# RocketFlash/EmbeddingNet

Measured on AMD Instinct MI355X. Metric: images/sec training (ResNet18, 224², triplet batch-hard) @ 1/2/4/8 GPU, higher is better.
Workload: dtype f32; 1 GPU; resnet18 224x224x3 synthetic U[0,1), 107-class P x K sampling, local batch 32x4=128 (139 resident batches cycled), E=256, margin 0.5, mining 'hardest' per local batch, radam, fp32 tensors (conv products on 16-bit MFMA from operand splits, fp32 accumulate: 3x3 stride-1 convs and their weight gradients, and the ResNets' other convs where both operands' ranges are known: two fp16 pieces + a per-tenso; global_batch=128, parallelism=dp1, active_triplets_min=192, dead_steps=0, resident_batches=139, step_mode=eager, mining=hardest

## Files before the change

embeddingnet_amd/csrc/conv.hip:

```cpp
#include "gemm_engine.h"
#include "conv_geom.h"
#include "../../include/embnet.h"
#include <stdlib.h>

namespace embnet {

struct InputTransform { const float* scale; const float* shift; int act; };
__device__ __forceinline__ float4 transform4(float4 v, bool ok, const float4& sc, const float4& sh, int act) {
  float4 z = make_float4(fmaf(v.x, sc.x, sh.x), fmaf(v.y, sc.y, sh.y), fmaf(v.z, sc.z, sh.z), fmaf(v.w, sc.w, sh.w));
  if (act == 1) {
    z = make_float4(fmaxf(z.x, 0.f), fmaxf(z.y, 0.f), fmaxf(z.z, 0.f), fmaxf(z.w, 0.f));
  } else if (act == 2) {
    z = make_float4(act_apply(2, z.x), act_apply(2, z.y), act_apply(2, z.z), act_apply(2, z.w));
  }
  return ok ? z : make_float4(0.f, 0.f, 0.f, 0.f);
}


template <int ROWS, bool VEC, bool TF = false>
struct LoadConvFwdA {
  using Tile = TileKC<ROWS>;
  static constexpr bool CAN_INTERLEAVE = VEC && !TF;
  Buf buf; int H, W, C, Kg; FastDiv dC, dS; int tid;
  unsigned base[Tile::PASSES]; int ih0[Tile::PASSES], iw0[Tile::PASSES];
// ... 268 lines not shown
#pragma unroll
      for (int r = 0; r < 16; ++r) acc[i][j][r] = (acc[i][j][r] * fb) * fa;
}

struct SplitTail { int n_full, parts, kt_part; float* ws; };

struct ConvFwdParams { const float* x; const float* w; const float* bias; float* y; ConvGeom g; int relu; SplitTail tail; const float* residual; InputTransform tf; float* stats; int stats_rows; int fair_from; Ranges rg; };

template <class G>
__device__ __forceinline__ void tail_decode(const SplitTail& t, int bid, int kt_total, int& tile, int& k0, int& k1,
                                            float*& part) {
  if (bid < t.n_full) { tile = xcd_remap(bid, t.n_full); k0 = 0; k1 = kt_total; part = nullptr; return; }
  const int j = bid - t.n_full;
  tile = t.n_full + j / t.parts;
  k0 = (j % t.parts) * t.kt_part; k1 = min(kt_total, k0 + t.kt_part);
  part = t.ws + (long)j * (G::BM * G::BN);
}

template <class G>
__device__ __forceinline__ void store_partial(const f32x16 (&acc)[G::TM][G::TN], float* smem, float* part) {
  for_each_acc_row4<G>(acc, smem, [&](int r, int c, float4 v) {
    *reinterpret_cast<float4*>(part + r * G::BN + c) = v;
  });
}


__device__ __forceinline__ void bn_sums_add(int act, float4 v, float4 xq, float4 sc, float4 sh, float4 mu, float4 rs,
                                            float4& s1, float4& s2, float4& s3) {
  float4 dz = v;
  if (act) {
    dz.x = act_grad(act, fmaf(xq.x, sc.x, sh.x), v.x); dz.y = act_grad(act, fmaf(xq.y, sc.y, sh.y), v.y);
    dz.z = act_grad(act, fmaf(xq.z, sc.z, sh.z), v.z); dz.w = act_grad(act, fmaf(xq.w, sc.w, sh.w), v.w);
  }
  s3.x = fmaxf(s3.x, fabsf(dz.x)); s3.y = fmaxf(s3.y, fabsf(dz.y)); s3.z = fmaxf(s3.z, fabsf(dz.z)); s3.w = fmaxf(s3.w, fabsf(dz.w));
  s1.x += dz.x; s1.y += dz.y; s1.z += dz.z; s1.w += dz.w;
  s2.x = fmaf(dz.x, (xq.x - mu.x) * rs.x, s2.x); s2.y = fmaf(dz.y, (xq.y - mu.y) * rs.y, s2.y);
  s2.z = fmaf(dz.z, (xq.z - mu.z) * rs.z, s2.z); s2.w = fmaf(dz.w, (xq.w - mu.w) * rs.w, s2.w);
}

__global__ __launch_bounds__(256) void tail_fixup_kernel(const float* __restrict__ ws, int parts, int bm, int bn, int wtm,
                                                         int n_full, int tiles_n, long m, int cols,
                                                         const float* __restrict__ bias, int relu,
                                                         const float* __restrict__ residual, float* __restrict__ out,
                                                         float* __restrict__ stats, int stats_rows, const BnSums bsum) {
  __shared__ float4 red[3][256];
  const int cpb = 1024 / wtm, qpb = cpb / 4;
  const int blocks_per_tile = bm * bn / 1024, col_groups = bn / cpb;
  const int t = blockIdx.x / blocks_per_tile, bi = blockIdx.x % blocks_per_tile;
  const int band = bi / col_groups, cg = bi % col_groups;
  const int rr = threadIdx.x / qpb, r = band * wtm + rr, c = cg * cpb + (threadIdx.x % qpb) * 4;
  const int tile = n_full + t;
  const long row = (long)(tile / tiles_n) * bm + r;
  const int col = (tile % tiles_n) * bn + c;
  const bool in = row < m && col < cols;
  float4 a = make_float4(0.f, 0.f, 0.f, 0.f);
  if (in) {
    const float* src = ws + (long)t * parts * bm * bn + r * bn + c;
    a = *reinterpret_cast<const float4*>(src);
    for (int k = 1; k < parts; ++k) {
      const float4 v = *reinterpret_cast<const float4*>(src + (long)k * bm * bn);
// ... 963 lines not shown
```

embeddingnet_amd/csrc/conv_geom.h:

```cpp
#pragma once
#include "common.h"

namespace embnet {

struct FastDiv {
  uint32_t mul, shift, d;
  static FastDiv make(uint32_t d) {
    FastDiv f; f.d = d;
    uint32_t s = 0; while ((1ull << s) < d) ++s;
    f.shift = s;
    f.mul = (uint32_t)((((1ull << s) - d) << 32) / d + 1);
    return f;
  }
  __device__ __forceinline__ uint32_t div(uint32_t n) const { return (__umulhi(n, mul) + n) >> shift; }
  __device__ __forceinline__ void divmod(uint32_t n, uint32_t& q, uint32_t& r) const { q = div(n); r = n - q * d; }
};

struct ConvGeom {
  int N, H, W, C, R, S, K, stride, pad_t, pad_l, OH, OW;
  FastDiv dOHW, dOW, dHW, dW, dC, dK, dS;
};

constexpr int ROW_INVALID = -(1 << 28);
constexpr size_t CONV_MAX_OPERAND_BYTES = 0x7FFFFFF0ull;


__device__ __forceinline__ void split_k(int kk, const FastDiv& dinner, const FastDiv& dS, int& r, int& s, int& c) {
  uint32_t rs, cc; dinner.divmod((uint32_t)kk, rs, cc);
  uint32_t rr, ss; dS.divmod(rs, rr, ss);
  r = (int)rr; s = (int)ss; c = (int)cc;
}

struct BnSums { const float* x; const float* scale; const float* shift; const float* mean; const float* rstd; int act; float* partial; int rows; int kinds; };
constexpr BnSums NO_BN_SUMS = BnSums{nullptr, nullptr, nullptr, nullptr, nullptr, 0, nullptr, 0};

void launch_tail_fixup(const float* ws, int parts, int bm, int bn, int wtm, int n_full, int rem, int tiles_n, long m, int cols,
                       const float* bias, int relu, const float* residual, float* out, float* stats, int stats_rows,
                       const BnSums& bsum, hipStream_t st);
void launch_slab_reduce(const float* slabs, int splits, long n, float* out, hipStream_t st);

bool thin_gemm_applies(int red, int ncols);
int thin_gemm_stats_rows(long m, int ncols);
int launch_thin_gemm(const float* in, const float* w, int w_transposed, long m, int red, int ncols, float* out, float* stats,
                     const float* bias, int relu, const float* residual, int stride, int n, int h, int wd, int oh, int ow, hipStream_t st);

bool thin_wgrad_applies(int c, int k);
int thin_wgrad_splits(long m, int c, int k);
int launch_thin_wgrad(const float* x, const float* dy, float* slabs, long m, int c, int k, int stride, int n, int h, int wd, int oh,
                      int ow, hipStream_t st);

inline int make_geom(ConvGeom& g, int n, int h, int w, int c, int r, int s, int k, int stride, int pad_t,
                     int pad_l, int oh, int ow, const char* who) {
  EMBNET_CHECK_ARG(n > 0 && h > 0 && w > 0 && c > 0 && r > 0 && s > 0 && k > 0 && stride > 0 && oh > 0 && ow > 0,
                   "%s: non-positive dimension", who);
  EMBNET_CHECK_ARG(pad_t >= 0 && pad_l >= 0, "%s: negative padding", who);
  EMBNET_CHECK_ARG((oh - 1) * stride + 1 - pad_t <= h && (ow - 1) * stride + 1 - pad_l <= w,
                   "%s: output %dx%d reaches outside the %dx%d input", who, oh, ow, h, w);
  EMBNET_CHECK_ARG((size_t)n * h * w * c * 4 <= CONV_MAX_OPERAND_BYTES && (size_t)n * oh * ow * k * 4 <= CONV_MAX_OPERAND_BYTES &&
// ... 12 lines not shown
```

embeddingnet_amd/csrc/conv_patch.hip:

```cpp
#include "gemm_engine.h"
#include "conv_geom.h"
#include "../../include/embnet.h"

namespace embnet {
namespace patch {

typedef __attribute__((address_space(3))) void* lds_ptr;
__device__ __forceinline__ void dma16(__amdgpu_buffer_rsrc_t r, unsigned char* lds, unsigned voff, unsigned soff) {
  __builtin_amdgcn_raw_ptr_buffer_load_lds(r, (lds_ptr)lds, 16, (int)voff, (int)soff, 0, 0);
}

template <int BN_>
struct GeomP {
  static constexpr int BM = 256, BN = BN_, WAVES_M = 4, WAVES_N = 2, WTM = 64, WTN = BN_ / 2, TM = 2, TN = WTN / 32;
};

struct PatchParams {
  const unsigned short* xp;
  const unsigned short* wp;
  float* y; const float* bias; const float* residual; float* stats; int stats_rows; int relu;
  ConvGeom g; unsigned x_plane_bytes, w_plane_bytes;
  int PH, PW; FastDiv dPHW, dPW;
  int LR;
  int n_full, parts, cc_part, n_pieces, grid; float* ws;
// ... 31 lines not shown
  kargp pp = kargs();
  FastDiv dOHW, dOW;
  dOHW.mul = pp->g.dOHW.mul; dOHW.shift = pp->g.dOHW.shift; dOHW.d = pp->g.dOHW.d;
  dOW.mul = pp->g.dOW.mul; dOW.shift = pp->g.dOW.shift; dOW.d = pp->g.dOW.d;
  uint32_t n, rem, oh, ow;
  dOHW.divmod((uint32_t)m, n, rem); dOW.divmod(rem, oh, ow);
  return (int)n * (pp->PH * pp->PW) + (int)oh * pp->PW + (int)ow;
}

template <class G, bool F16, int NP>
__device__ __forceinline__ void step_planes(const bf16x8 (&a)[G::TM][NP], const bf16x8 (&b)[G::TN][NP], f32x16 (&acc)[G::TM][G::TN]) {
  if constexpr (F16) {
    f16x8 ah[G::TM][2], bh[G::TN][2];
#pragma unroll
    for (int i = 0; i < G::TM; ++i) { ah[i][0] = __builtin_bit_cast(f16x8, a[i][0]); ah[i][1] = __builtin_bit_cast(f16x8, a[i][1]); }
#pragma unroll
    for (int i = 0; i < G::TN; ++i) { bh[i][0] = __builtin_bit_cast(f16x8, b[i][0]); bh[i][1] = __builtin_bit_cast(f16x8, b[i][1]); }
    mfma_step_h<G::TM, G::TN>(ah, bh, acc);
  } else {
    mfma_step3<G>(a, b, acc);
  }
}

template <class G, int BN, bool BNS, bool F16>
__device__ __forceinline__ void patch_epilogue(const PatchParams& p, const Item& cur, f32x16 (&acc)[G::TM][G::TN], int M, int K,
                                               int wave, int lane, int h, int wm, int wn) {
  constexpr int TM = G::TM, TN = G::TN;
  if (F16) {
    const float osx = p.a_range ? scale_pair(scale_exponent_of(__uint_as_float(*p.a_range))).y
                                : planes_scale_slot(p.xp, (long)(p.x_plane_bytes >> 1))[1];
    const float osw = planes_scale_slot(p.wp, (long)(p.w_plane_bytes >> 1))[1];
#pragma unroll
    for (int im = 0; im < TM; ++im)
#pragma unroll
      for (int in = 0; in < TN; ++in)
#pragma unroll
        for (int rr = 0; rr < 16; ++rr) acc[im][in][rr] = (acc[im][in][rr] * osw) * osx;
  }
  if (cur.part) {
    float* part = cur.part + (wm + 4 * h) * BN + wn + (lane & 31);
#pragma unroll
    for (int im = 0; im < TM; ++im)
#pragma unroll
      for (int in = 0; in < TN; ++in)
#pragma unroll
        for (int rr = 0; rr < 16; ++rr)
          part[(im * 32 + (rr & 3) + 8 * (rr >> 2)) * BN + in * 32] = acc[im][in][rr];
  } else {
    const bool inner = cur.m0 + 256 <= M && cur.n0 + BN <= K;
#pragma unroll
    for (int in = 0; in < TN; ++in) {
      const int col = cur.n0 + wn + in * 32 + (lane & 31);
      const bool cok = col < K;
      const float bv = (p.bias && cok) ? p.bias[col] : 0.f;
      float s1 = 0.f, s2 = 0.f;
      constexpr bool bnm = BNS;
      float bsc = 0.f, bsh = 0.f, bmu = 0.f, brs = 0.f;
      float ev[BNS ? TM : 1][16];
      if (BNS) {
        if (cok) { bsc = p.bn.scale[col]; bsh = p.bn.shift[col]; bmu = p.bn.mean[col]; brs = p.bn.rstd[col]; }
#pragma unroll
        for (int im = 0; im < TM; ++im) {
          const long o0 = (long)(cur.m0 + wm + im * 32 + 4 * h) * K + col;
#pragma unroll
          for (int rr = 0; rr < 16; ++rr) {
            const int row = cur.m0 + wm + im * 32 + (rr & 3) + 8 * (rr >> 2) + 4 * h;
            ev[BNS ? im : 0][rr] = (inner || (row < M && cok)) ? p.bn.x[o0 + (long)((rr & 3) + 8 * (rr >> 2)) * K] : 0.f;
          }
        }
      }
#pragma unroll
      for (int im = 0; im < TM; ++im) {
        const long o0 = (long)(cur.m0 + wm + im * 32 + 4 * h) * K + col;
        float v[16];
#pragma unroll
        for (int rr = 0; rr < 16; ++rr) { v[rr] = acc[im][in][rr] + bv; if (p.relu) v[rr] = fmaxf(v[rr], 0.f); }
        if (inner) {
          if (p.residual) {
#pragma unroll
            for (int rr = 0; rr < 16; ++rr) v[rr] += p.residual[o0 + (long)((rr & 3) + 8 * (rr >> 2)) * K];
          }
#pragma unroll
          for (int rr = 0; rr < 16; ++rr) {
            p.y[o0 + (long)((rr & 3) + 8 * (rr >> 2)) * K] = v[rr];
            if (BNS) {
              const float e = ev[BNS ? im : 0][rr], dz = act_grad(p.bn.act, fmaf(e, bsc, bsh), v[rr]);
              s1 += dz; s2 = fmaf(dz, (e - bmu) * brs, s2);
            } else { s1 += v[rr]; s2 = fmaf(v[rr], v[rr], s2); }
          }
        } else {
#pragma unroll
          for (int rr = 0; rr < 16; ++rr) {
            const int row = cur.m0 + wm + im * 32 + (rr & 3) + 8 * (rr >> 2) + 4 * h;
            if (row < M && cok) {
              const long o = o0 + (long)((rr & 3) + 8 * (rr >> 2)) * K;
              if (p.residual) v[rr] += p.residual[o];
              p.y[o] = v[rr];
              if (BNS) {
                const float e = ev[BNS ? im : 0][rr], dz = act_grad(p.bn.act, fmaf(e, bsc, bsh), v[rr]);
                s1 += dz; s2 = fmaf(dz, (e - bmu) * brs, s2);
              } else { s1 += v[rr]; s2 = fmaf(v[rr], v[rr], s2); }
            }
          }
        }
      }
      if (p.stats || bnm) {
        s1 += __shfl_xor(s1, 32, 64); s2 += __shfl_xor(s2, 32, 64);
        if (h == 0 && cok) {
          float* const dst = bnm ? p.bn.partial : p.stats;
          const long prow = (long)cur.tile_m * G::WAVES_M + wave / G::WAVES_N, P = bnm ? p.bn.rows : p.stats_rows;
          dst[(long)col * P + prow] = s1;
          dst[((long)K + col) * P + prow] = s2;
        }
      }
    }
  }

}

template <int BN, int R, int S, int TPS, int NBS, bool BNS = false, bool F16 = false, bool PIPE = false>
__global__ __launch_bounds__(640) void conv_patch_kernel(const PatchParams p) {
  using G = GeomP<BN>;
  constexpr int NP = F16 ? 2 : 3;
  constexpr int TM = G::TM, TN = G::TN, SPC = R * S / TPS, D = NBS - 1;
  constexpr int SBY = TPS * NP * BN * 32;
  constexpr int NBI = TPS * NP * (BN / 32);
  static_assert((R * S) % TPS == 0 && SPC >= 2, "steps per chunk");
  extern __shared__ __attribute__((aligned(16))) unsigned char smem[];
  const int tid = threadIdx.x, lane = tid & 63, h = lane >> 5;
  const int wave = __builtin_amdgcn_readfirstlane(tid >> 6);
  const int LR = p.LR, PLP = LR * 32, PB = NP * PLP;
  unsigned char* const bslot0 = smem + 2 * PB;
  const int b = blockIdx.x;
  const int n_mine = b < p.n_full ? (p.n_full - b + p.grid - 1) / p.grid : 0;
  const int n_items = n_mine + (b < p.n_pieces ? 1 : 0);
  if (n_items == 0) return;
  const int dhalf = (lane & 1) ^ ((lane >> 4) & 1);

  if (wave == 8) {
    const __amdgpu_buffer_rsrc_t wr = __builtin_amdgcn_make_buffer_rsrc(const_cast<unsigned short*>(p.wp), 0, 3u * p.w_plane_bytes, 0x00020000);
    const int K = p.g.K, NCC = p.g.C / 16;
    const unsigned wpb = p.w_plane_bytes;
    int it = 0; Item t = work_item<BN>(0, n_mine);
    int cc = t.cc_b, st = 0; bool live = true;
// ... 16 lines not shown
        for (int q = 0; q < NP; ++q)
#pragma unroll
          for (int gb = 0; gb < BN / 32; ++gb)
            dma16(wr, slot + ((tp * NP + q) * BN + gb * 32) * 32, live ? rowoff[gb] : OOB, q * wpb + so);
      }
      if (live && ++st == SPC) {
        st = 0;
        if (++cc == t.cc_e) {
          if (++it < n_items) { t = work_item<BN>(it, n_mine); cc = t.cc_b; tile_rows(); } else live = false;
        }
      }
    };
    int total = 0;
    for (int i = 0; i < n_items; ++i) { const Item q = work_item<BN>(i, n_mine); total += (q.cc_e - q.cc_b) * SPC; }
    for (int gs = 0; gs < D; ++gs) issue(gs);
    for (int gs = 0; gs < total; ++gs) {
      asm volatile("s_waitcnt vmcnt(%0)" :: "n"((D - 1) * NBI) : "memory");
      __builtin_amdgcn_s_barrier();
      issue(gs + D);
    }
    asm volatile("s_waitcnt vmcnt(0)" ::: "memory");
    return;
  }
  if (wave == 9) {
    const __amdgpu_buffer_rsrc_t xr = __builtin_amdgcn_make_buffer_rsrc(const_cast<unsigned short*>(p.xp), 0, 3u * p.x_plane_bytes, 0x00020000);
    const int NG = LR / 32;
    const unsigned xpb = p.x_plane_bytes, chunk_bytes = 32u * (unsigned)(p.g.N * p.g.H * p.g.W);
    unsigned poff[16];
    auto tile_offsets = [&](const Item& t) {
      kargp pp = kargs();
      FastDiv dPHW, dPW;
      dPHW.mul = pp->dPHW.mul; dPHW.shift = pp->dPHW.shift; dPHW.d = pp->dPHW.d;
      dPW.mul = pp->dPW.mul; dPW.shift = pp->dPW.shift; dPW.d = pp->dPW.d;
      const int P0 = padded_pos(t.m0), N = pp->g.N, H = pp->g.H, W = pp->g.W, pt = pp->g.pad_t, pl = pp->g.pad_l;
#pragma unroll
      for (int gI = 0; gI < 16; ++gI) {
        const int idx = P0 + 32 * gI + (lane >> 1);
        uint32_t n, rem, py, px;
        dPHW.divmod((uint32_t)idx, n, rem); dPW.divmod(rem, py, px);
        const int ih = (int)py - pt, iw = (int)px - pl;
        const bool ok = gI < NG && (int)n < N && (unsigned)ih < (unsigned)H && (unsigned)iw < (unsigned)W;
        poff[gI] = ok ? 32u * (unsigned)(((int)n * H + ih) * W + iw) + 16u * dhalf : OOB;
      }
    };
    auto issue = [&](int cc, int gc) {
      unsigned char* buf = smem + (gc & 1) * PB;
// ... 106 lines not shown
          const int tap = st * TPS + tp, r = tap / S, s = tap % S;
          bf16x8 a[TM][NP], bb[TN][NP];
#pragma unroll
          for (int im = 0; im < TM; ++im) {
            const int idx = rowidx[im] + r * PW + s;
            const unsigned char* ap = pbuf + idx * 32 + ((h ^ ((idx >> 3) & 1)) << 4);
#pragma unroll
            for (int q = 0; q < NP; ++q) a[im][q] = *reinterpret_cast<const bf16x8*>(ap + q * PLP);
          }
#pragma unroll
          for (int in = 0; in < TN; ++in) {
            const int row = wn + in * 32 + (lane & 31);
            const unsigned char* bp = bs + (tp * NP * BN + row) * 32 + ((h ^ ((row >> 3) & 1)) << 4);
#pragma unroll
            for (int q = 0; q < NP; ++q) bb[in][q] = *reinterpret_cast<const bf16x8*>(bp + q * BN * 32);
          }
          step_planes<G, F16>(a, bb, acc);
          if (TPS > 1) __builtin_amdgcn_sched_barrier(0);
        }
        ++gs;
      }
      ++gc;
    }
    patch_epilogue<G, BN, BNS, F16>(p, cur, acc, M, K, wave, lane, h, wm, wn);
  }
}

template <int BN, int G, int NS, bool F16>
__global__ __launch_bounds__(704) void conv1x1_planes_kernel(const PatchParams p) {
  using GP = GeomP<BN>;
  static_assert(F16, "the 1x1 planes kernel is built for the two-piece fp16 format");
  constexpr int NP = 2, TM = GP::TM, TN = GP::TN, D = NS - 1;
  constexpr int A_BYTES = G * NP * 256 * 32, B_BYTES = G * NP * BN * 32, STAGE = A_BYTES + B_BYTES;
  constexpr int NBI_B = G * NP * (BN / 32), NBI_A = NP * 8;
  extern __shared__ __attribute__((aligned(16))) unsigned char smem[];
  const int tid = threadIdx.x, lane = tid & 63, h = lane >> 5;
  const int wave = __builtin_amdgcn_readfirstlane(tid >> 6);
  const int b = blockIdx.x;
  const int n_mine = b < p.n_full ? (p.n_full - b + p.grid - 1) / p.grid : 0;
  const int n_items = n_mine + (b < p.n_pieces ? 1 : 0);
  if (n_items == 0) return;
  const int dhalf = (lane & 1) ^ ((lane >> 4) & 1);
  int total = 0;
  for (int i = 0; i < n_items; ++i) { const Item q = work_item<BN, 16 * G>(i, n_mine); total += q.cc_e - q.cc_b; }

  if (wave >= 8) {
    const bool is_b = wave == 8;
    const int tp = wave - 9;
// ... 89 lines not shown
        for (int q = 0; q < 2; ++q) {
#pragma unroll
          for (int im = 0; im < TM; ++im) a[im][q] = *reinterpret_cast<const f16x8*>(sa + (c2 * NP + q) * 256 * 32 + aoff[im]);
#pragma unroll
          for (int in = 0; in < TN; ++in) bb[in][q] = *reinterpret_cast<const f16x8*>(sb + (c2 * NP + q) * BN * 32 + boff[in]);
        }
      };
      load(0, fa[0], fb[0]);
      __builtin_amdgcn_sched_barrier(0);
#pragma unroll
      for (int c2 = 0; c2 < G; ++c2) {
        if (c2 + 1 < G) load(c2 + 1, fa[(c2 + 1) & 1], fb[(c2 + 1) & 1]);
        mfma_step_h<TM, TN>(fa[c2 & 1], fb[c2 & 1], acc);
        constexpr int NMF = 3 * TM * TN, NRD = 2 * (TM + TN);
#pragma unroll
        for (int i = 0; i < NMF; ++i) {
          __builtin_amdgcn_sched_group_barrier(0x008, 1, 0);
          if (c2 + 1 < G && i < NRD) __builtin_amdgcn_sched_group_barrier(0x100, 1, 0);
        }
        __builtin_amdgcn_sched_barrier(0);
      }
      ++gs;
    }
    patch_epilogue<GP, BN, false, F16>(p, cur, acc, M, K, wave, lane, h, wm, wn);
  }
}

template <int BN>
__global__ __launch_bounds__(704) void conv1x1_a32_kernel(const PatchParams p) {
  using GP = GeomP<BN>;
  constexpr int G = 2, NS = 3, NP = 2, TM = GP::TM, TN = GP::TN, D = NS - 1;
  constexpr int A_BYTES = 256 * 128, B_BYTES = G * NP * BN * 32, STAGE = A_BYTES + B_BYTES;
  constexpr int NBI_B = G * NP * (BN / 32), NBI_A = 16;
  extern __shared__ __attribute__((aligned(16))) unsigned char smem[];
  const int tid = threadIdx.x, lane = tid & 63, h = lane >> 5;
  const int wave = __builtin_amdgcn_readfirstlane(tid >> 6);
  const int b = blockIdx.x;
  const int n_mine = b < p.n_full ? (p.n_full - b + p.grid - 1) / p.grid : 0;
  const int n_items = n_mine + (b < p.n_pieces ? 1 : 0);
  if (n_items == 0) return;
  int total = 0;
  for (int i = 0; i < n_items; ++i) { const Item q = work_item<BN, 16 * G>(i, n_mine); total += q.cc_e - q.cc_b; }

  if (wave >= 8) {
    const bool is_b = wave == 8;
    const int tp = wave - 9;
    const __amdgpu_buffer_rsrc_t rs = is_b
// ... 98 lines not shown
        for (int q = 0; q < 2; ++q)
#pragma unroll
          for (int in = 0; in < TN; ++in) bb[in][q] = *reinterpret_cast<const f16x8*>(sb + (c2 * NP + q) * BN * 32 + boff[in]);
      };
      auto split = [&](f16x8 (&a)[TM][2]) {
        typedef uint32_t u32x4 __attribute__((ext_vector_type(4)));
#pragma unroll
        for (int im = 0; im < TM; ++im) {
          const Split4H s0 = split4h(raw[im][0], a_scale), s1 = split4h(raw[im][1], a_scale);
          a[im][0] = __builtin_bit_cast(f16x8, u32x4{s0.p[0].x, s0.p[0].y, s1.p[0].x, s1.p[0].y});
          a[im][1] = __builtin_bit_cast(f16x8, u32x4{s0.p[1].x, s0.p[1].y, s1.p[1].x, s1.p[1].y});
        }
      };
      load_raw(0); load_b(0, fb[0]);
      split(fa[0]);
#pragma unroll
      for (int c2 = 0; c2 < G; ++c2) {
        if (c2 + 1 < G) { load_raw(c2 + 1); load_b(c2 + 1, fb[(c2 + 1) & 1]); }
        mfma_step_h<TM, TN>(fa[c2 & 1], fb[c2 & 1], acc);
        if (c2 + 1 < G) split(fa[(c2 + 1) & 1]);
      }
      ++gs;
    }
    patch_epilogue<GP, BN, false, true>(p, cur, acc, M, K, wave, lane, h, wm, wn);
  }
}

struct WPlanesTensor { const float* w; unsigned short* out; int R, S, C, K, flip, pad; };
static_assert(sizeof(WPlanesTensor) == 40, "descriptor layout is part of the ABI (include/embnet.h)");
__global__ __launch_bounds__(256) void weight_planes_kernel(const WPlanesTensor* __restrict__ table, const int* __restrict__ chunks, int f16) {
  const WPlanesTensor t = table[chunks[2 * blockIdx.x]];
  const int rows = t.flip ? t.C : t.K, red = t.flip ? t.K : t.C, ncc = red / 16;
  const long plane = (long)t.R * t.S * t.C * t.K, total4 = plane / 4;
  const long i = (long)chunks[2 * blockIdx.x + 1] * 1024 + threadIdx.x;
#pragma unroll
  for (int u = 0; u < 4; ++u) {
    const long i4 = i + u * 256;
    if (i4 >= total4) return;
    long e = 4 * i4;
    const int j = (int)(e % 16); e /= 16;
    const int row = (int)(e % rows); e /= rows;
    const int s = (int)(e % t.S); e /= t.S;
    const int cc = (int)(e % ncc); const int r = (int)(e / ncc);
    float v[4];
#pragma unroll
    for (int q = 0; q < 4; ++q) {
      const int ch = cc * 16 + j + q;
// ... 227 lines not shown
                              void* workspace, size_t workspace_bytes, void* stream, const char* who) {
  const ConvGeom& g = p.g;
  const long M = (long)g.N * g.OH * g.OW;
  p.stats_rows = cdiv(M, 256) * 4;
  p.grid = pl.grid;
  if (pl.n_pieces > 0 && (pl.ws_bytes > workspace_bytes || !workspace)) { pl.n_full = pl.tiles; pl.n_pieces = 0; pl.parts = 1; }
  p.n_full = pl.n_full; p.parts = pl.parts; p.cc_part = pl.cc_part; p.n_pieces = pl.n_pieces; p.ws = (float*)workspace;
  hipStream_t st = (hipStream_t)stream;
  {
    EMBNET_TRACE_FLOP(kname, 2.0 * M * g.K * g.R * g.S * g.C, operand_bytes + 4.0 * (double)M * g.K * (p.residual ? 2 : 1), st);
    launch(p, pl, st);
  }
  if (p.n_pieces > 0)
    launch_tail_fixup(p.ws, p.parts, 256, pl.bn, 64, p.n_full, pl.tiles - p.n_full, cdiv(g.K, pl.bn), M, g.K, p.bias, p.relu, p.residual,
                      p.y, p.stats, p.stats_rows, p.bn, st);
  return check_launch(who);
}

template <int BN, int TPS, int NBS>
static void launch_patch_as(const PatchParams& p, size_t lds, hipStream_t st) {
  if (!p.bn.x) {
    if (planes_f16()) launch_planes<conv_patch_kernel<BN, 3, 3, TPS, NBS, false, true, true>>(p, 640, lds, st);
    else launch_planes<conv_patch_kernel<BN, 3, 3, TPS, NBS, false, false>>(p, 640, lds, st);
  } else if (!planes_f16()) launch_planes<conv_patch_kernel<BN, 3, 3, TPS, NBS, true, false>>(p, 640, lds, st);
  else launch_planes<conv_patch_kernel<BN, 3, 3, TPS, NBS, true, true>>(p, 640, lds, st);
}
static void launch_patch(const PatchParams& p, const Plan& pl, hipStream_t st) {
  if (pl.bn == 128 && pl.tps == 3) { if (pl.nbs == 3) launch_patch_as<128, 3, 3>(p, pl.lds, st); else launch_patch_as<128, 3, 2>(p, pl.lds, st); }
  else if (pl.bn == 128) { if (pl.nbs == 6) launch_patch_as<128, 1, 6>(p, pl.lds, st); else launch_patch_as<128, 1, 4>(p, pl.lds, st); }
  else launch_patch_as<64, 3, 3>(p, pl.lds, st);
}

static int conv2d_patch_impl(const void* xp, const void* wp, const float* bias, float* y, int n, int h, int wd, int c,
                             int r, int s, int k, int pad_t, int pad_l, int oh, int ow, int relu,
                             const float* residual, float* stats, const BnSums& bsum, void* workspace, size_t workspace_bytes,
                             void* stream) {
  EMBNET_CHECK_ARG(xp && wp && y, "conv2d_patch: null pointer");
  EMBNET_CHECK_ARG(r == 3 && s == 3, "conv2d_patch: 3x3 kernels (1x1: embnet_conv2d_planes1x1_f32)");
  Plan pl;
  EMBNET_CHECK_ARG(make_plan(n, c, r, s, k, 1, oh, ow, pl), "conv2d_patch: unsupported geometry (see embnet_conv2d_patch_supported)");
  PatchParams p{(const unsigned short*)xp, (const unsigned short*)wp, y, bias, residual, stats, 0, relu};
  if (int rc = make_geom(p.g, n, h, wd, c, r, s, k, 1, pad_t, pad_l, oh, ow, "conv2d_patch")) return rc;
  p.x_plane_bytes = (unsigned)((size_t)n * h * wd * c * 2);
  p.w_plane_bytes = (unsigned)((size_t)r * s * c * k * 2);
  p.PH = oh + r - 1; p.PW = ow + s - 1;
  p.dPHW = FastDiv::make(p.PH * p.PW); p.dPW = FastDiv::make(p.PW);
  p.LR = pl.LR;
  p.bn = bsum;
  static thread_local char kname[160];
  snprintf(kname, sizeof kname, "void embnet::patch::conv_patch_kernel<%d, 3, 3, %d, %d, %s%s>(embnet::patch::PatchParams)", pl.bn, pl.tps, pl.nbs,
           p.bn.x ? "true" : "false", planes_f16() ? (p.bn.x ? ", true" : ", true, true") : "");
  return launch_planes_gemm(p, pl, kname, (planes_f16() ? 4.0 : 6.0) * ((double)n * h * wd * c + (double)r * s * c * k), launch_patch,
                            workspace, workspace_bytes, stream, "conv2d_patch");
}

extern "C" int embnet_conv2d_patch_f32(const void* xp, const void* wp, const float* bias, float* y, int n, int h, int wd, int c,
                                       int r, int s, int k, int pad_t, int pad_l, int oh, int ow, int relu,
                                       const float* residual, float* stats, void* workspace, size_t workspace_bytes,
                                       void* stream) {
  return conv2d_patch_impl(xp, wp, bias, y, n, h, wd, c, r, s, k, pad_t, pad_l, oh, ow, relu, residual, stats, NO_BN_SUMS, workspace,
                           workspace_bytes, stream);
}

static void fill_1x1(PatchParams& p) {
  const ConvGeom& g = p.g;
  p.w_plane_bytes = (unsigned)((size_t)g.C * g.K * 2);
  p.PH = g.OH; p.PW = g.OW; p.dPHW = FastDiv::make(g.OH * g.OW); p.dPW = FastDiv::make(g.OW);
  p.LR = 256;
  p.bn = NO_BN_SUMS;
}

static void launch_1x1(const PatchParams& p, const Plan& pl, hipStream_t st) {
  if (pl.bn == 128) launch_planes<conv1x1_planes_kernel<128, ONE_G, ONE_NS, true>>(p, 704, pl.lds, st);
  else launch_planes<conv1x1_planes_kernel<64, ONE_G, ONE_NS, true>>(p, 704, pl.lds, st);
// ... 22 lines not shown
  else launch_planes<conv1x1_a32_kernel<64>>(p, 704, pl.lds, st);
}
extern "C" int embnet_conv2d_dma1x1_supported(int n, int h, int wd, int c, int k, int stride, int oh, int ow) {
  Plan pl;
  return dma1x1_ok(n, h, wd, c, k, stride, oh, ow, pl) ? 1 : 0;
}
extern "C" int embnet_conv2d_dma1x1_f32(const float* x, const void* wp, const float* bias, float* y, int n, int h, int wd, int c, int k,
                                        int stride, int oh, int ow, int relu, const float* residual, float* stats,
                                        const uint32_t* x_range, void* workspace, size_t workspace_bytes, void* stream) {
  EMBNET_CHECK_ARG(x && wp && y && x_range, "conv2d_dma1x1: null pointer (the activation's range slot is required)");
  EMBNET_CHECK_ARG(!(reinterpret_cast<uintptr_t>(x) & 15) && !(reinterpret_cast<uintptr_t>(x_range) & 3), "conv2d_dma1x1: alignment");
  Plan pl;
  EMBNET_CHECK_ARG(dma1x1_ok(n, h, wd, c, k, stride, oh, ow, pl), "conv2d_dma1x1: unsupported geometry (embnet_conv2d_dma1x1_supported)");
  PatchParams p{(const unsigned short*)x, (const unsigned short*)wp, y, bias, residual, stats, 0, relu};
  if (int rc = make_geom(p.g, n, h, wd, c, 1, 1, k, stride, 0, 0, oh, ow, "conv2d_dma1x1")) return rc;
  p.x_plane_bytes = 0; p.x32_bytes = (unsigned)((size_t)n * h * wd * c * 4); p.a_range = x_range;
  fill_1x1(p);
  static thread_local char kname[160];
  snprintf(kname, sizeof kname, "void embnet::patch::conv1x1_a32_kernel<%d>(embnet::patch::PatchParams)", pl.bn);
  return launch_planes_gemm(p, pl, kname, 4.0 * ((double)n * oh * ow * c + (double)c * k), launch_dma1x1, workspace, workspace_bytes, stream,
                            "conv2d_dma1x1");
}

extern "C" int embnet_conv2d_patch_bnsums_f32(const void* xp, const void* wp, float* y, int n, int h, int wd, int c, int r, int s, int k,
                                              int pad_t, int pad_l, int oh, int ow, const float* bn_x, const float* bn_scale,
                                              const float* bn_shift, const float* bn_mean, const float* bn_rstd, int bn_act,
                                              float* bn_partial, int bn_rows, void* workspace, size_t workspace_bytes, void* stream) {
  EMBNET_CHECK_ARG(bn_x && bn_scale && bn_shift && bn_mean && bn_rstd && bn_partial, "conv2d_patch_bnsums: null pointer");
  EMBNET_CHECK_ARG(bn_act >= 0 && bn_act <= 2, "conv2d_patch_bnsums: activation code %d", bn_act);
  EMBNET_CHECK_ARG(bn_rows > 0 && bn_rows == embnet_conv2d_patch_stats_rows(n, oh, ow),
                   "conv2d_patch_bnsums: rows %d for this geometry (see embnet_conv2d_patch_stats_rows)", bn_rows);
  return conv2d_patch_impl(xp, wp, nullptr, y, n, h, wd, c, r, s, k, pad_t, pad_l, oh, ow, 0, nullptr, nullptr,
                           BnSums{bn_x, bn_scale, bn_shift, bn_mean, bn_rstd, bn_act, bn_partial, bn_rows}, workspace, workspace_bytes, stream);
}
```

embeddingnet_amd/layers.py:

```python
import contextlib
import math
import os as _os

import torch
from torch import nn

from . import _lib
from ._lib import check, ptr, stream


def env_switch(var, default):
    return {"0": False, "1": True}.get(_os.environ.get(var), default)


@contextlib.contextmanager
def switches(**values):
    old = {name: globals()[name][0] for name in values}
    try:
        for name, v in values.items():
            globals()[name][0] = v
        yield
    finally:
        for name, v in old.items():
            globals()[name][0] = v
# ... 448 lines not shown
    return base.as_strided(tuple(shape), (0,) * len(shape), 1)


def _is_placeholder(t):
    return (t.dim() == 4 and t.numel() > 1 and t.stride() == (0, 0, 0, 0) and t.storage_offset() == 1
            and t.untyped_storage().nbytes() == 12)


def _take_dy_planes(dy):
    e = DY_PLANES.pop(dy.data_ptr(), None)
    return e[0] if (e is not None and e[1].shape == dy.shape) else None


def patch_ok(n, h, wd, c, r, s, k, stride, oh, ow):
    return bool(_lib.lib().embnet_conv2d_patch_supported(n, c, r, s, k, stride, oh, ow))


def _patch_dgrad(dy_planes, w, dx, n, h, wd, c, r, s, k, pt, pl, oh, ow, dx_add, bn_src=None):
    lib = _lib.lib()
    ws = workspace(lib.embnet_conv2d_patch_workspace_bytes(n, k, r, s, c, h, wd), dx.device)
    if bn_src is not None and dx_add is None and PATCH_BN_SUMS[0]:
        bn_x, bn_stats, bn_act = bn_src
        rows = lib.embnet_conv2d_patch_stats_rows(n, h, wd)
        partial = torch.empty((2, c, rows), device=dx.device, dtype=torch.float32)
        st = _StatsRows(bn_stats)
        check(lib.embnet_conv2d_patch_bnsums_f32(ptr(dy_planes), ptr(weight_planes(w, 1)), ptr(dx), n, oh, ow, k, r, s, c,
                                                 r - 1 - pt, s - 1 - pl, h, wd, ptr(bn_x), st.scale, st.shift, st.mean, st.rstd,
                                                 int(bn_act), ptr(partial), rows, ptr(ws), ws.numel() * 4, stream()))
        BN_SUMS.put(dx.data_ptr(), (partial, rows, bn_x.data_ptr(), dx.detach()), 8, "oldest")
        return
    check(lib.embnet_conv2d_patch_f32(ptr(dy_planes), ptr(weight_planes(w, 1)), None, ptr(dx), n, oh, ow, k, r, s, c,
                                      r - 1 - pt, s - 1 - pl, h, wd, 0, ptr(dx_add), None, ptr(ws), ws.numel() * 4, stream()))


STATS_ROWS = ("mean", "rstd", "scale", "shift", "bound", "range", "xhat")
STATS_HEIGHTS = (4, 6, 7)


class _StatsRows:
    __slots__ = STATS_ROWS

    def __init__(self, stats):
        p, height, row = stats.data_ptr(), stats.shape[0], 4 * stats.shape[1]
        self.mean, self.rstd, self.scale, self.shift = p, p + row, p + 2 * row, p + 3 * row
        self.bound, self.range = (p + 4 * row, p + 5 * row) if height >= 6 else (None, None)
        self.xhat = p + 6 * row if height >= 7 else None


def _in_affine(in_stats):
    st = _StatsRows(in_stats) if in_stats is not None else None
    return (st.scale, st.shift) if st is not None else (None, None)
# ... 1689 lines not shown
```

include/embnet.h:

```cpp
#ifndef EMBNET_H
#define EMBNET_H

#include <stddef.h>
#include <stdint.h>

#ifdef __cplusplus
extern "C" {
#endif

#define EMBNET_ABI_VERSION 22

enum {
  EMBNET_MINE_SEMIHARD = 0,
  EMBNET_MINE_HARDEST = 1,
  EMBNET_MINE_RANDOM_HARD = 2,
  EMBNET_MINE_BATCH_HARD = 3
};

int embnet_abi_version(void);
const char* embnet_last_error(void);

int embnet_trace_enable(int on);
int embnet_trace_reset(void);
int embnet_trace_count(void);
// ... 143 lines not shown
int embnet_conv1x1_thin_supported(int red, int ncols);

int embnet_conv2d_patch_supported(int n, int c, int r, int s, int k, int stride, int oh, int ow);
size_t embnet_conv2d_patch_workspace_bytes(int n, int c, int r, int s, int k, int oh, int ow);
int embnet_conv2d_patch_stats_rows(int n, int oh, int ow);
int embnet_conv2d_patch_f32(const void* x_planes, const void* w_planes, const float* bias, float* y, int n, int h, int wd, int c,
                            int r, int s, int k, int pad_t, int pad_l, int oh, int ow, int relu, const float* residual,
                            float* stats, void* workspace, size_t workspace_bytes, void* stream);
int embnet_conv2d_stem_supported(int n, int h, int wd, int c, int r, int s, int k, int stride, int pad_t, int pad_l, int oh, int ow);
int embnet_conv2d_stem_stats_rows(int n, int oh, int ow);
int embnet_conv2d_stem_f32(const float* x, const float* w, float* y, int n, int h, int wd, int pad_t, int pad_l, int oh, int ow,
                           float* stats, const uint32_t* x_range, const uint32_t* w_range, void* stream);
int embnet_conv2d_planes1x1_f32(const void* x_planes, const void* w_planes, const float* bias, float* y, int n, int h, int wd, int c,
                                int k, int stride, int oh, int ow, int relu, const float* residual, float* stats,
                                void* workspace, size_t workspace_bytes, void* stream);
int embnet_conv2d_dma1x1_supported(int n, int h, int wd, int c, int k, int stride, int oh, int ow);
int embnet_conv2d_dma1x1_f32(const float* x, const void* wp, const float* bias, float* y, int n, int h, int wd, int c, int k,
                             int stride, int oh, int ow, int relu, const float* residual, float* stats, const uint32_t* x_range,
                             void* workspace, size_t workspace_bytes, void* stream);
int embnet_conv2d_patch_bnsums_f32(const void* x_planes, const void* w_planes, float* y, int n, int h, int wd, int c, int r, int s,
                                   int k, int pad_t, int pad_l, int oh, int ow, const float* bn_x, const float* bn_scale,
                                   const float* bn_shift, const float* bn_mean, const float* bn_rstd, int bn_act,
                                   float* bn_partial, int bn_rows, void* workspace, size_t workspace_bytes, void* stream);
int embnet_se_mlp_supported(int n, int c, int s);
int embnet_se_mlp_fwd(const float* pooled, const float* w1, const float* b1, const float* w2, const float* b2, int n, int c, int s,
                      float* z1, float* gate, void* stream);
int embnet_se_mlp_bwd(const float* dgate, const float* gate, const float* z1, const float* pooled, const float* w1, const float* w2,
                      int n, int c, int s, float* dz1, float* dpooled, float* dw1, float* db1, float* dw2, float* db2, void* stream);
int embnet_planes_from_f32(const float* x, long pixels, int c, void* planes, void* stream);
int embnet_conv_weight_planes_chunk_elems(void);
int embnet_conv_weight_planes(const void* table, int n_tensors, const int32_t* chunks, int n_chunks, void* stream);
int embnet_affine_act_planes(const float* x, long m, int c, const float* scale, const float* shift, int act, float* y,
                             void* planes, void* stream);
int embnet_affine_act_planes_ex(const float* x, long m, int c, const float* scale, const float* shift, int act, float* y,
                                void* planes, const float* y_bound, uint32_t* y_range, void* stream);
int embnet_conv2d_wgrad_planes_supported(int n, int h, int wd, int c, int r, int s, int k, int stride, int pad_t, int pad_l,
                                         int oh, int ow);
int embnet_conv2d_wgrad_planes_splits(int n, int h, int wd, int c, int k);
size_t embnet_conv2d_wgrad_planes_workspace_bytes(int n, int h, int wd, int c, int k);
int embnet_conv2d_wgrad_planes_f32(const void* x_planes, const void* dy_planes, float* dw, void* workspace,
                                   size_t workspace_bytes, int n, int h, int wd, int c, int k, int reduce, void* stream);

int embnet_u8_to_f32(const void* src, const int32_t* index, int n, long pixels, int c_in, int c_out, float denom, float* dst,
                     void* stream);

size_t embnet_augment_param_floats(void);
// ... 257 lines not shown
```

Before: 16820 images/sec.

## Move BN-backward sums out of patch conv epilogue into dedicated sums waves

The fused dgrad+BN-sums patch kernel no longer computes batch-norm backward reductions inside the MFMA waves' epilogue. Two extra waves (768 threads) stream back the freshly written dx tile plus the BN input and accumulate sum, weighted sum and a new max|dz| statistic, running one tile behind the compute waves. The aim is to take the extra reads and ALU work off the GEMM critical path and overlap them with the next tile's math. The cost is more barriers and higher register and occupancy pressure. It also adds a third partial-stats plane that the Python caller now allocates and requests.

```diff
diff --git a/embeddingnet_amd/csrc/conv.hip b/embeddingnet_amd/csrc/conv.hip
--- a/embeddingnet_amd/csrc/conv.hip
+++ b/embeddingnet_amd/csrc/conv.hip
@@ -314,20 +314,6 @@
   for_each_acc_row4<G>(acc, smem, [&](int r, int c, float4 v) {
     *reinterpret_cast<float4*>(part + r * G::BN + c) = v;
   });
-}
-
-
-__device__ __forceinline__ void bn_sums_add(int act, float4 v, float4 xq, float4 sc, float4 sh, float4 mu, float4 rs,
-                                            float4& s1, float4& s2, float4& s3) {
-  float4 dz = v;
-  if (act) {
-    dz.x = act_grad(act, fmaf(xq.x, sc.x, sh.x), v.x); dz.y = act_grad(act, fmaf(xq.y, sc.y, sh.y), v.y);
-    dz.z = act_grad(act, fmaf(xq.z, sc.z, sh.z), v.z); dz.w = act_grad(act, fmaf(xq.w, sc.w, sh.w), v.w);
-  }
-  s3.x = fmaxf(s3.x, fabsf(dz.x)); s3.y = fmaxf(s3.y, fabsf(dz.y)); s3.z = fmaxf(s3.z, fabsf(dz.z)); s3.w = fmaxf(s3.w, fabsf(dz.w));
-  s1.x += dz.x; s1.y += dz.y; s1.z += dz.z; s1.w += dz.w;
-  s2.x = fmaf(dz.x, (xq.x - mu.x) * rs.x, s2.x); s2.y = fmaf(dz.y, (xq.y - mu.y) * rs.y, s2.y);
-  s2.z = fmaf(dz.z, (xq.z - mu.z) * rs.z, s2.z); s2.w = fmaf(dz.w, (xq.w - mu.w) * rs.w, s2.w);
 }
 
 __global__ __launch_bounds__(256) void tail_fixup_kernel(const float* __restrict__ ws, int parts, int bm, int bn, int wtm,
diff --git a/embeddingnet_amd/csrc/conv_geom.h b/embeddingnet_amd/csrc/conv_geom.h
--- a/embeddingnet_amd/csrc/conv_geom.h
+++ b/embeddingnet_amd/csrc/conv_geom.h
@@ -34,6 +34,19 @@
 struct BnSums { const float* x; const float* scale; const float* shift; const float* mean; const float* rstd; int act; float* partial; int rows; int kinds; };
 constexpr BnSums NO_BN_SUMS = BnSums{nullptr, nullptr, nullptr, nullptr, nullptr, 0, nullptr, 0};
 
+__device__ __forceinline__ void bn_sums_add(int act, float4 v, float4 xq, float4 sc, float4 sh, float4 mu, float4 rs,
+                                            float4& s1, float4& s2, float4& s3) {
+  float4 dz = v;
+  if (act) {
+    dz.x = act_grad(act, fmaf(xq.x, sc.x, sh.x), v.x); dz.y = act_grad(act, fmaf(xq.y, sc.y, sh.y), v.y);
+    dz.z = act_grad(act, fmaf(xq.z, sc.z, sh.z), v.z); dz.w = act_grad(act, fmaf(xq.w, sc.w, sh.w), v.w);
+  }
+  s3.x = fmaxf(s3.x, fabsf(dz.x)); s3.y = fmaxf(s3.y, fabsf(dz.y)); s3.z = fmaxf(s3.z, fabsf(dz.z)); s3.w = fmaxf(s3.w, fabsf(dz.w));
+  s1.x += dz.x; s1.y += dz.y; s1.z += dz.z; s1.w += dz.w;
+  s2.x = fmaf(dz.x, (xq.x - mu.x) * rs.x, s2.x); s2.y = fmaf(dz.y, (xq.y - mu.y) * rs.y, s2.y);
+  s2.z = fmaf(dz.z, (xq.z - mu.z) * rs.z, s2.z); s2.w = fmaf(dz.w, (xq.w - mu.w) * rs.w, s2.w);
+}
+
 void launch_tail_fixup(const float* ws, int parts, int bm, int bn, int wtm, int n_full, int rem, int tiles_n, long m, int cols,
                        const float* bias, int relu, const float* residual, float* out, float* stats, int stats_rows,
                        const BnSums& bsum, hipStream_t st);
diff --git a/embeddingnet_amd/csrc/conv_patch.hip b/embeddingnet_amd/csrc/conv_patch.hip
--- a/embeddingnet_amd/csrc/conv_patch.hip
+++ b/embeddingnet_amd/csrc/conv_patch.hip
@@ -77,7 +77,7 @@
   }
 }
 
-template <class G, int BN, bool BNS, bool F16>
+template <class G, int BN, bool F16>
 __device__ __forceinline__ void patch_epilogue(const PatchParams& p, const Item& cur, f32x16 (&acc)[G::TM][G::TN], int M, int K,
                                                int wave, int lane, int h, int wm, int wn) {
   constexpr int TM = G::TM, TN = G::TN;
@@ -109,21 +109,6 @@
       const bool cok = col < K;
       const float bv = (p.bias && cok) ? p.bias[col] : 0.f;
       float s1 = 0.f, s2 = 0.f;
-      constexpr bool bnm = BNS;
-      float bsc = 0.f, bsh = 0.f, bmu = 0.f, brs = 0.f;
-      float ev[BNS ? TM : 1][16];
-      if (BNS) {
-        if (cok) { bsc = p.bn.scale[col]; bsh = p.bn.shift[col]; bmu = p.bn.mean[col]; brs = p.bn.rstd[col]; }
-#pragma unroll
-        for (int im = 0; im < TM; ++im) {
-          const long o0 = (long)(cur.m0 + wm + im * 32 + 4 * h) * K + col;
-#pragma unroll
-          for (int rr = 0; rr < 16; ++rr) {
-            const int row = cur.m0 + wm + im * 32 + (rr & 3) + 8 * (rr >> 2) + 4 * h;
-            ev[BNS ? im : 0][rr] = (inner || (row < M && cok)) ? p.bn.x[o0 + (long)((rr & 3) + 8 * (rr >> 2)) * K] : 0.f;
-          }
-        }
-      }
 #pragma unroll
       for (int im = 0; im < TM; ++im) {
         const long o0 = (long)(cur.m0 + wm + im * 32 + 4 * h) * K + col;
@@ -138,10 +123,7 @@
 #pragma unroll
           for (int rr = 0; rr < 16; ++rr) {
             p.y[o0 + (long)((rr & 3) + 8 * (rr >> 2)) * K] = v[rr];
-            if (BNS) {
-              const float e = ev[BNS ? im : 0][rr], dz = act_grad(p.bn.act, fmaf(e, bsc, bsh), v[rr]);
-              s1 += dz; s2 = fmaf(dz, (e - bmu) * brs, s2);
-            } else { s1 += v[rr]; s2 = fmaf(v[rr], v[rr], s2); }
+            s1 += v[rr]; s2 = fmaf(v[rr], v[rr], s2);
           }
         } else {
 #pragma unroll
@@ -151,19 +133,16 @@
               const long o = o0 + (long)((rr & 3) + 8 * (rr >> 2)) * K;
               if (p.residual) v[rr] += p.residual[o];
               p.y[o] = v[rr];
-              if (BNS) {
-                const float e = ev[BNS ? im : 0][rr], dz = act_grad(p.bn.act, fmaf(e, bsc, bsh), v[rr]);
-                s1 += dz; s2 = fmaf(dz, (e - bmu) * brs, s2);
-              } else { s1 += v[rr]; s2 = fmaf(v[rr], v[rr], s2); }
+              s1 += v[rr]; s2 = fmaf(v[rr], v[rr], s2);
             }
           }
         }
       }
-      if (p.stats || bnm) {
+      if (p.stats) {
         s1 += __shfl_xor(s1, 32, 64); s2 += __shfl_xor(s2, 32, 64);
         if (h == 0 && cok) {
-          float* const dst = bnm ? p.bn.partial : p.stats;
-          const long prow = (long)cur.tile_m * G::WAVES_M + wave / G::WAVES_N, P = bnm ? p.bn.rows : p.stats_rows;
+          float* const dst = p.stats;
+          const long prow = (long)cur.tile_m * G::WAVES_M + wave / G::WAVES_N, P = p.stats_rows;
           dst[(long)col * P + prow] = s1;
           dst[((long)K + col) * P + prow] = s2;
         }
@@ -173,8 +152,134 @@
 
 }
 
+constexpr int SUMS_G = 2, SUMS_PD = 3;
+
+template <int BN, int SPC>
+__device__ __forceinline__ void sums_wave(const PatchParams& p, int sw, int lane, int n_mine, int n_items) {
+  constexpr int QPR = BN / 4, RPL = 64 / QPR, NU = 128 / RPL, NS = SUMS_PD + 1, G = SUMS_G;
+  static_assert(NU % G == 0, "whole ring slots per tile");
+  const int q = lane % QPR, rl = lane / QPR;
+  const int K = p.g.K, M = p.g.N * p.g.OH * p.g.OW;
+  Buf yb, eb;
+  yb.init(p.y, 0); eb.init(p.bn.x, 0);
+  const unsigned ustride = (unsigned)(RPL * K) * 4u;
+  const int act = p.bn.act;
+  const float4 zero4 = make_float4(0.f, 0.f, 0.f, 0.f);
+  bool cok = false;
+  int tile_m = 0, col = 0, next_u = NU;
+  unsigned voff[G];
+#pragma unroll
+  for (int j = 0; j < G; ++j) voff[j] = OOB;
+  float4 sc = zero4, sh = zero4, mu = zero4, rs = zero4, acc[2][3];
+  float4 yv[NS][G], ev[NS][G];
+#pragma unroll
+  for (int i = 0; i < NS; ++i)
+#pragma unroll
+    for (int j = 0; j < G; ++j) yv[i][j] = ev[i][j] = zero4;
+
+  auto begin = [&](const Item& t) __attribute__((always_inline)) {
+    tile_m = t.tile_m; col = t.n0 + 4 * q; cok = col < K;
+#pragma unroll
+    for (int j = 0; j < G; ++j)
+      voff[j] = cok ? ((unsigned)(t.m0 + 128 * sw + rl + j * RPL) * (unsigned)K + (unsigned)col) * 4u : OOB;
+    const size_t end = (size_t)min(M, t.m0 + 128 * sw + 128) * K * 4;
+    yb.init(p.y, end); eb.init(p.bn.x, end);
+    const int cc = cok ? col : 0;
+    sc = *reinterpret_cast<const float4*>(p.bn.scale + cc); sh = *reinterpret_cast<const float4*>(p.bn.shift + cc);
+    mu = *reinterpret_cast<const float4*>(p.bn.mean + cc); rs = *reinterpret_cast<const float4*>(p.bn.rstd + cc);
+    next_u = 0;
+#pragma unroll
+    for (int b = 0; b < 2; ++b)
+#pragma unroll
+      for (int k = 0; k < 3; ++k) acc[b][k] = zero4;
+    asm volatile("" :: "v"(sc.w), "v"(sh.w), "v"(mu.w), "v"(rs.w));
+  };
+  auto issue = [&](int slot) __attribute__((always_inline)) {
+#pragma unroll
+    for (int j = 0; j < G; ++j) {
+      yv[slot][j] = yb.ld4(voff[j]); ev[slot][j] = eb.ld4(voff[j]);
+      voff[j] += G * ustride;
+    }
+    next_u = min(next_u + G, NU);
+  };
+  auto finish = [&]() __attribute__((always_inline)) {
+    float* const dst = p.bn.partial;
+    const long P = p.bn.rows;
+#pragma unroll
+    for (int b = 0; b < 2; ++b) {
+      float4 s1 = acc[b][0], s2 = acc[b][1], s3 = acc[b][2];
+#pragma unroll
+      for (int o = QPR; o < 64; o <<= 1) {
+        s1.x += __shfl_xor(s1.x, o, 64); s1.y += __shfl_xor(s1.y, o, 64); s1.z += __shfl_xor(s1.z, o, 64); s1.w += __shfl_xor(s1.w, o, 64);
+        s2.x += __shfl_xor(s2.x, o, 64); s2.y += __shfl_xor(s2.y, o, 64); s2.z += __shfl_xor(s2.z, o, 64); s2.w += __shfl_xor(s2.w, o, 64);
+        s3.x = fmaxf(s3.x, __shfl_xor(s3.x, o, 64)); s3.y = fmaxf(s3.y, __shfl_xor(s3.y, o, 64));
+        s3.z = fmaxf(s3.z, __shfl_xor(s3.z, o, 64)); s3.w = fmaxf(s3.w, __shfl_xor(s3.w, o, 64));
+      }
+      if (rl == 0 && cok) {
+        const long prow = (long)tile_m * 4 + 2 * sw + b;
+        float* d1 = dst + (long)col * P + prow;
+        asm volatile("" : "+v"(d1));
+        float* d2 = d1 + (long)K * P;
+        d1[0] = s1.x; d1[P] = s1.y; d1[2 * P] = s1.z; d1[3 * P] = s1.w;
+        d2[0] = s2.x; d2[P] = s2.y; d2[2 * P] = s2.z; d2[3 * P] = s2.w;
+        if (p.bn.kinds == 3) {
+          float* d3 = d2 + (long)K * P;
+          d3[0] = s3.x; d3[P] = s3.y; d3[2 * P] = s3.z; d3[3 * P] = s3.w;
+        }
+      }
+    }
+  };
+  auto consume = [&](int slot) __attribute__((always_inline)) {
+    float4& a1 = acc[slot & 1][0]; float4& a2 = acc[slot & 1][1]; float4& a3 = acc[slot & 1][2];
+    auto add = [&](int a) __attribute__((always_inline)) {
+#pragma unroll
+      for (int j = 0; j < G; ++j) {
+        bn_sums_add(a, yv[slot][j], ev[slot][j], sc, sh, mu, rs, a1, a2, a3);
+        __builtin_amdgcn_sched_barrier(0);
+      }
+    };
+    if (act == 2) add(2); else if (act == 1) add(1); else add(0);
+#pragma unroll
+    for (int j = 0; j < G; ++j) yv[slot][j] = zero4;
+  };
+
+  bool have = false;
+  Item prev = work_item<BN>(0, n_mine);
+  for (int it = 0; it <= n_items; ++it) {
+    const bool closing = it == n_items;
+    const Item t = work_item<BN>(closing ? 0 : it, n_mine);
+    const int steps = closing ? 1 : (t.cc_e - t.cc_b) * SPC;
+    __builtin_amdgcn_s_barrier();
+    __builtin_amdgcn_fence(__ATOMIC_ACQUIRE, "workgroup");
+    if (have) begin(prev);
+#pragma unroll 1
+    for (int st0 = 0; st0 < steps; st0 += NS) {
+#pragma unroll
+      for (int j = 0; j < NS; ++j)
+        if (st0 + j < steps) {
+          issue(j); consume((j + 1) % NS);
+          if (st0 + j + 1 < steps) __builtin_amdgcn_s_barrier();
+        }
+    }
+    if (have) {
+#pragma unroll
+      for (int i = 0; i < NS; ++i) consume(i);
+#pragma unroll 1
+      while (next_u < NU) {
+#pragma unroll
+        for (int i = 0; i < NS; ++i) issue(i);
+#pragma unroll
+        for (int i = 0; i < NS; ++i) consume(i);
+      }
+      finish();
+      next_u = NU; yb.init(p.y, 0); eb.init(p.bn.x, 0);
+    }
+    have = !closing && !t.part; prev = t;
+  }
+}
+
 template <int BN, int R, int S, int TPS, int NBS, bool BNS = false, bool F16 = false, bool PIPE = false>
-__global__ __launch_bounds__(640) void conv_patch_kernel(const PatchParams p) {
+__global__ __launch_bounds__(BNS ? 768 : 640) void conv_patch_kernel(const PatchParams p) {
   using G = GeomP<BN>;
   constexpr int NP = F16 ? 2 : 3;
   constexpr int TM = G::TM, TN = G::TN, SPC = R * S / TPS, D = NBS - 1;
@@ -237,6 +342,9 @@
     asm volatile("s_waitcnt vmcnt(0)" ::: "memory");
     return;
   }
+  if constexpr (BNS) {
+    if (wave >= 10) { sums_wave<BN, SPC>(p, wave - 10, lane, n_mine, n_items); return; }
+  }
   if (wave == 9) {
     const __amdgpu_buffer_rsrc_t xr = __builtin_amdgcn_make_buffer_rsrc(const_cast<unsigned short*>(p.xp), 0, 3u * p.x_plane_bytes, 0x00020000);
     const int NG = LR / 32;
@@ -389,8 +497,9 @@
       }
       ++gc;
     }
-    patch_epilogue<G, BN, BNS, F16>(p, cur, acc, M, K, wave, lane, h, wm, wn);
-  }
+    patch_epilogue<G, BN, F16>(p, cur, acc, M, K, wave, lane, h, wm, wn);
+  }
+  if constexpr (BNS) __syncthreads();
 }
 
 template <int BN, int G, int NS, bool F16>
@@ -526,7 +635,7 @@
       }
       ++gs;
     }
-    patch_epilogue<GP, BN, false, F16>(p, cur, acc, M, K, wave, lane, h, wm, wn);
+    patch_epilogue<GP, BN, F16>(p, cur, acc, M, K, wave, lane, h, wm, wn);
   }
 }
 
@@ -671,7 +780,7 @@
       }
       ++gs;
     }
-    patch_epilogue<GP, BN, false, true>(p, cur, acc, M, K, wave, lane, h, wm, wn);
+    patch_epilogue<GP, BN, true>(p, cur, acc, M, K, wave, lane, h, wm, wn);
   }
 }
 
@@ -945,8 +1054,8 @@
   if (!p.bn.x) {
     if (planes_f16()) launch_planes<conv_patch_kernel<BN, 3, 3, TPS, NBS, false, true, true>>(p, 640, lds, st);
     else launch_planes<conv_patch_kernel<BN, 3, 3, TPS, NBS, false, false>>(p, 640, lds, st);
-  } else if (!planes_f16()) launch_planes<conv_patch_kernel<BN, 3, 3, TPS, NBS, true, false>>(p, 640, lds, st);
-  else launch_planes<conv_patch_kernel<BN, 3, 3, TPS, NBS, true, true>>(p, 640, lds, st);
+  } else if (planes_f16()) launch_planes<conv_patch_kernel<BN, 3, 3, TPS, NBS, true, true, true>>(p, 768, lds, st);
+  else launch_planes<conv_patch_kernel<BN, 3, 3, TPS, NBS, true, false>>(p, 768, lds, st);
 }
 static void launch_patch(const PatchParams& p, const Plan& pl, hipStream_t st) {
   if (pl.bn == 128 && pl.tps == 3) { if (pl.nbs == 3) launch_patch_as<128, 3, 3>(p, pl.lds, st); else launch_patch_as<128, 3, 2>(p, pl.lds, st); }
@@ -972,7 +1081,7 @@
   p.bn = bsum;
   static thread_local char kname[160];
   snprintf(kname, sizeof kname, "void embnet::patch::conv_patch_kernel<%d, 3, 3, %d, %d, %s%s>(embnet::patch::PatchParams)", pl.bn, pl.tps, pl.nbs,
-           p.bn.x ? "true" : "false", planes_f16() ? (p.bn.x ? ", true" : ", true, true") : "");
+           p.bn.x ? "true" : "false", planes_f16() ? ", true, true" : "");
   return launch_planes_gemm(p, pl, kname, (planes_f16() ? 4.0 : 6.0) * ((double)n * h * wd * c + (double)r * s * c * k), launch_patch,
                             workspace, workspace_bytes, stream, "conv2d_patch");
 }
@@ -1041,14 +1150,26 @@
                             "conv2d_dma1x1");
 }
 
+extern "C" int embnet_conv2d_patch_bnsums_f32_ex(const void* xp, const void* wp, float* y, int n, int h, int wd, int c, int r, int s, int k,
+                                                 int pad_t, int pad_l, int oh, int ow, const float* bn_x, const float* bn_scale,
+                                                 const float* bn_shift, const float* bn_mean, const float* bn_rstd, int bn_act,
+                                                 float* bn_partial, int bn_rows, int kinds, void* workspace, size_t workspace_bytes,
+                                                 void* stream) {
+  EMBNET_CHECK_ARG(bn_x && bn_scale && bn_shift && bn_mean && bn_rstd && bn_partial && y, "conv2d_patch_bnsums: null pointer");
+  EMBNET_CHECK_ARG(bn_act >= 0 && bn_act <= 2, "conv2d_patch_bnsums: activation code %d", bn_act);
+  EMBNET_CHECK_ARG(kinds == 2 || kinds == 3, "conv2d_patch_bnsums: kinds %d (2: the sums, 3: + max |dz|)", kinds);
+  EMBNET_CHECK_ARG(bn_rows > 0 && bn_rows == embnet_conv2d_patch_stats_rows(n, oh, ow),
+                   "conv2d_patch_bnsums: rows %d for this geometry (see embnet_conv2d_patch_stats_rows)", bn_rows);
+  EMBNET_CHECK_ARG(!((reinterpret_cast<uintptr_t>(y) | reinterpret_cast<uintptr_t>(bn_x) | reinterpret_cast<uintptr_t>(bn_scale) |
+                      reinterpret_cast<uintptr_t>(bn_shift) | reinterpret_cast<uintptr_t>(bn_mean) | reinterpret_cast<uintptr_t>(bn_rstd)) & 15),
+                   "conv2d_patch_bnsums: operands must be 16-byte aligned");
+  return conv2d_patch_impl(xp, wp, nullptr, y, n, h, wd, c, r, s, k, pad_t, pad_l, oh, ow, 0, nullptr, nullptr,
+                           BnSums{bn_x, bn_scale, bn_shift, bn_mean, bn_rstd, bn_act, bn_partial, bn_rows, kinds}, workspace, workspace_bytes, stream);
+}
 extern "C" int embnet_conv2d_patch_bnsums_f32(const void* xp, const void* wp, float* y, int n, int h, int wd, int c, int r, int s, int k,
                                               int pad_t, int pad_l, int oh, int ow, const float* bn_x, const float* bn_scale,
                                               const float* bn_shift, const float* bn_mean, const float* bn_rstd, int bn_act,
                                               float* bn_partial, int bn_rows, void* workspace, size_t workspace_bytes, void* stream) {
-  EMBNET_CHECK_ARG(bn_x && bn_scale && bn_shift && bn_mean && bn_rstd && bn_partial, "conv2d_patch_bnsums: null pointer");
-  EMBNET_CHECK_ARG(bn_act >= 0 && bn_act <= 2, "conv2d_patch_bnsums: activation code %d", bn_act);
-  EMBNET_CHECK_ARG(bn_rows > 0 && bn_rows == embnet_conv2d_patch_stats_rows(n, oh, ow),
-                   "conv2d_patch_bnsums: rows %d for this geometry (see embnet_conv2d_patch_stats_rows)", bn_rows);
-  return conv2d_patch_impl(xp, wp, nullptr, y, n, h, wd, c, r, s, k, pad_t, pad_l, oh, ow, 0, nullptr, nullptr,
-                           BnSums{bn_x, bn_scale, bn_shift, bn_mean, bn_rstd, bn_act, bn_partial, bn_rows}, workspace, workspace_bytes, stream);
-}
+  return embnet_conv2d_patch_bnsums_f32_ex(xp, wp, y, n, h, wd, c, r, s, k, pad_t, pad_l, oh, ow, bn_x, bn_scale, bn_shift, bn_mean, bn_rstd,
+                                           bn_act, bn_partial, bn_rows, 2, workspace, workspace_bytes, stream);
+}
diff --git a/embeddingnet_amd/layers.py b/embeddingnet_amd/layers.py
--- a/embeddingnet_amd/layers.py
+++ b/embeddingnet_amd/layers.py
@@ -494,11 +494,11 @@
     if bn_src is not None and dx_add is None and PATCH_BN_SUMS[0]:
         bn_x, bn_stats, bn_act = bn_src
         rows = lib.embnet_conv2d_patch_stats_rows(n, h, wd)
-        partial = torch.empty((2, c, rows), device=dx.device, dtype=torch.float32)
+        partial = torch.empty((3, c, rows), device=dx.device, dtype=torch.float32)
         st = _StatsRows(bn_stats)
-        check(lib.embnet_conv2d_patch_bnsums_f32(ptr(dy_planes), ptr(weight_planes(w, 1)), ptr(dx), n, oh, ow, k, r, s, c,
-                                                 r - 1 - pt, s - 1 - pl, h, wd, ptr(bn_x), st.scale, st.shift, st.mean, st.rstd,
-                                                 int(bn_act), ptr(partial), rows, ptr(ws), ws.numel() * 4, stream()))
+        check(lib.embnet_conv2d_patch_bnsums_f32_ex(ptr(dy_planes), ptr(weight_planes(w, 1)), ptr(dx), n, oh, ow, k, r, s, c,
+                                                    r - 1 - pt, s - 1 - pl, h, wd, ptr(bn_x), st.scale, st.shift, st.mean, st.rstd,
+                                                    int(bn_act), ptr(partial), rows, 3, ptr(ws), ws.numel() * 4, stream()))
         BN_SUMS.put(dx.data_ptr(), (partial, rows, bn_x.data_ptr(), dx.detach()), 8, "oldest")
         return
     check(lib.embnet_conv2d_patch_f32(ptr(dy_planes), ptr(weight_planes(w, 1)), None, ptr(dx), n, oh, ow, k, r, s, c,
diff --git a/include/embnet.h b/include/embnet.h
--- a/include/embnet.h
+++ b/include/embnet.h
@@ -189,6 +189,10 @@
                                    int k, int pad_t, int pad_l, int oh, int ow, const float* bn_x, const float* bn_scale,
                                    const float* bn_shift, const float* bn_mean, const float* bn_rstd, int bn_act,
                                    float* bn_partial, int bn_rows, void* workspace, size_t workspace_bytes, void* stream);
+int embnet_conv2d_patch_bnsums_f32_ex(const void* x_planes, const void* w_planes, float* y, int n, int h, int wd, int c, int r, int s,
+                                      int k, int pad_t, int pad_l, int oh, int ow, const float* bn_x, const float* bn_scale,
+                                      const float* bn_shift, const float* bn_mean, const float* bn_rstd, int bn_act,
+                                      float* bn_partial, int bn_rows, int kinds, void* workspace, size_t workspace_bytes, void* stream);
 int embnet_se_mlp_supported(int n, int c, int s);
 int embnet_se_mlp_fwd(const float* pooled, const float* w1, const float* b1, const float* w2, const float* b2, int n, int c, int s,
                       float* z1, float* gate, void* stream);
```

Result: no change. 16810 images/sec (median of 2 runs) (-0.0%).
